# wheretrue/exon

Measured on AMD Instinct MI355X. Metric: Mrows/sec filter+agg on 1B-row synthetic VCF; achieved HBM GB/s vs peak, higher is better.
Workload: dtype f64

## Files before the change

exon_amd/csrc/kernels.h:

```cpp
#pragma once
#include <hip/hip_runtime.h>
#include <stdint.h>

namespace exon {

struct Workspace {
  unsigned long long* partials = nullptr;
  size_t partial_capacity = 0;
  int* status = nullptr;
  uint2* tail_rec_a = nullptr;
  uint2* tail_rec_b = nullptr;
  size_t tail_capacity = 0;
  unsigned* tail_u32 = nullptr;
};

struct LaunchCfg {
  int compute_units = 256;
  int blocks_per_cu = 8;
  bool overwrite = false;
  bool x_is_int = false;
  bool y_is_int = false;
};

size_t k2_partial_words(const LaunchCfg&);
// ... 14 lines not shown
                                int64_t region_start, int64_t region_end, int64_t* d_count, bool strict = false);

hipError_t launch_flag_mapq_group_count(hipStream_t s, const LaunchCfg& cfg, const Workspace& ws, const int32_t* flag,
                                        const uint8_t* flag_valid, const uint8_t* mapq, const uint8_t* mapq_valid,
                                        const int32_t* ref_id, const uint8_t* ref_valid, int64_t n, int32_t flag_mask,
                                        int32_t flag_value, int32_t mapq_min, int32_t n_refs, int64_t* d_counts);

hipError_t launch_cmp_avg_by_group(hipStream_t s, const LaunchCfg& cfg, const Workspace& ws, const float* x,
                                   const uint8_t* x_valid, const float* y, const uint8_t* y_valid, const int32_t* gid,
                                   int64_t n, double thr, int cmp_op, int n_groups, int64_t* d_counts, double* d_sums);

hipError_t launch_cmp_minmax_by_group(hipStream_t s, const LaunchCfg& cfg, const Workspace& ws, const float* x,
                                      const uint8_t* x_valid, const float* y, const uint8_t* y_valid, const int32_t* gid,
                                      int64_t n, double thr, int cmp_op, int n_groups, int64_t* d_state);

hipError_t launch_qual_pos_hist(hipStream_t s, const LaunchCfg& cfg, const Workspace& ws, const int32_t* offsets,
                                const uint8_t* bytes, int64_t n_reads, int lmax, int64_t* d_hist);
hipError_t launch_qual_pos_hist_views(hipStream_t s, const LaunchCfg& cfg, const Workspace& ws, const int32_t* starts,
                                      const int32_t* ends, const uint8_t* bytes, int64_t n_reads, int lmax,
                                      int64_t* d_hist);

constexpr int K5_MAX_CHUNKS = 64;
struct K5Chunks {
  const int32_t* off[K5_MAX_CHUNKS];
  const int32_t* ends[K5_MAX_CHUNKS];
  const uint8_t* bytes[K5_MAX_CHUNKS];
  int64_t n[K5_MAX_CHUNKS];
  int count;
};
hipError_t launch_qual_pos_hist_chunks(hipStream_t s, const LaunchCfg& cfg, const Workspace& ws, const K5Chunks& ch, int lmax,
                                       int64_t* d_hist);

constexpr int K9_LEN_LDS = 8192;
constexpr int64_t read_stats_words(int lmax) { return 4 + ((int64_t)lmax + 1) + 102 + 257; }
hipError_t launch_read_stats_hist(hipStream_t s, const LaunchCfg& cfg, const Workspace& ws, const uint8_t* sbytes, const int32_t* ss,
                                  const int32_t* se, const uint8_t* qbytes, const int32_t* qs, const int32_t* qe, int64_t n_reads, int lmax,
                                  int64_t* d_state);

hipError_t launch_region_mask(hipStream_t s, bool range_form, const int32_t* id_col, const uint8_t* id_valid, const int64_t* start,
                              const int64_t* end, const uint8_t* pos_valid, const uint8_t* in_valid, int64_t n, int32_t id,
                              int64_t a, int64_t b, uint8_t* out_valid, unsigned long long* n_pass);

hipError_t launch_value_mask(hipStream_t s, const void* x, const uint8_t* x_valid, bool x_is_int, double literal, int cmp_op, const uint8_t* region_mask,
                             const uint8_t* in_valid, int64_t n, uint8_t* out_valid, unsigned long long* n_pass);

hipError_t launch_flag_mapq_mask(hipStream_t s, const int32_t* flag, const uint8_t* mapq, const uint8_t* mapq_valid, int32_t flag_mask, int32_t flag_value,
                                 int32_t mapq_min, const uint8_t* region_mask, const uint8_t* in_valid, int64_t n, uint8_t* out_valid, unsigned long long* n_pass);

hipError_t launch_fold_states(hipStream_t s, const void* gathered, int world, int64_t n_i64, int64_t n_f64, void* out, int64_t n_max = 0);

hipError_t launch_permute_add_state(hipStream_t s, const void* src, void* dst, const int32_t* map, int n_map, int G, int planes_i64,
                                    int tail_i64, int planes_f64, int planes_max);

hipError_t launch_read_probe(hipStream_t s, const LaunchCfg& cfg, const void* const* buffers, int n_buffers, int64_t bytes_each,
                             unsigned* sink);

hipError_t launch_gen_c2(hipStream_t s, uint64_t seed, int64_t n_total, int64_t lo, int64_t hi, int32_t* chrom,
                         int64_t* pos);
hipError_t launch_gen_c3(hipStream_t s, uint64_t seed, int64_t lo, int64_t hi, int32_t* flag, uint8_t* mapq,
                         uint8_t* mapq_valid, int32_t* ref_id, uint8_t* ref_valid);
hipError_t launch_gen_c4(hipStream_t s, uint64_t seed, int64_t lo, int64_t hi, float* af, uint8_t* af_valid,
                         float* qual, uint8_t* qual_valid, int32_t* filter_id);
hipError_t launch_gen_c6(hipStream_t s, uint64_t seed, int64_t lo, int64_t hi, int32_t* ref_id, uint8_t* ref_valid,
                         int64_t* start, int64_t* end, uint8_t* pos_valid);
hipError_t launch_gen_c5(hipStream_t s, uint64_t seed, int64_t lo, int64_t hi, int32_t read_len, int32_t* offsets,
                         uint8_t* bytes);

}
```

exon_amd/csrc/kernels.hip:

```cpp
#include "kernels.h"
#include "host/cmp_key.h"

#include <algorithm>
#include <cstdlib>
#include <cstring>
#include <mutex>
#include <type_traits>

namespace exon {

struct ShapeBig {
  static constexpr int THREADS = 1024, J = 4;
};
struct ShapeSmall {
  static constexpr int THREADS = 256, J = 2;
};
struct ShapeBigJ2 {
  static constexpr int THREADS = 1024, J = 2;
};
template <typename S>
struct ShapeOf {
  static constexpr int WAVES = S::THREADS / 64;
  static constexpr int WAVE_TILE = 256 * S::J;
  static constexpr int TILE = WAVES * WAVE_TILE;
// ... 209 lines not shown
    for (int r = 0; r < world; ++r) t = max(t, gathered[(size_t)r * V + v]);
    out[v] = t;
  } else if (v < n_i64) {
    unsigned long long t = 0;
    for (int r = 0; r < world; ++r) t += gathered[(size_t)r * V + v];
    out[v] = t;
  } else {
    double t = 0.0;
    for (int r = 0; r < world; ++r) t += __longlong_as_double((long long)gathered[(size_t)r * V + v]);
    out[v] = (unsigned long long)__double_as_longlong(t);
  }
}

hipError_t launch_fold_states(hipStream_t s, const void* gathered, int world, int64_t n_i64, int64_t n_f64, void* out, int64_t n_max) {
  const int64_t V = n_i64 + n_f64;
  if (V <= 0 || world < 1 || n_max < 0 || n_max > n_i64) return hipErrorInvalidValue;
  hipLaunchKernelGGL(fold_states, dim3((unsigned)((V + 255) / 256)), dim3(256), 0, s,
                     static_cast<const unsigned long long*>(gathered), world, (int)V, (int)n_i64, (int)n_max,
                     static_cast<unsigned long long*>(out));
  return hipGetLastError();
}

__global__ __launch_bounds__(256) void permute_add_state(const unsigned long long* __restrict__ src, unsigned long long* __restrict__ dst,
                                                         const int32_t* __restrict__ map, int n_map, int G, int planes_i64, int tail_i64,
                                                         int planes_f64, int planes_max) {
  const int g = blockIdx.x * 256 + threadIdx.x;
  if (g < tail_i64) {
    const size_t w = (size_t)planes_i64 * G + g;
    if (src[w]) atomicAdd(&dst[w], src[w]);
  }
  if (g >= n_map || g >= G) return;
  const int t = map[g];
  if (t < 0 || t >= G) return;
  for (int p = 0; p < planes_i64; ++p) {
    const unsigned long long v = src[(size_t)p * G + g];
    if (!v) continue;
    if (p >= planes_i64 - planes_max) atomicMax(&dst[(size_t)p * G + t], v);
    else atomicAdd(&dst[(size_t)p * G + t], v);
  }
  const size_t fbase = (size_t)planes_i64 * G + tail_i64;
  for (int p = 0; p < planes_f64; ++p) {
    const double v = __longlong_as_double((long long)src[fbase + (size_t)p * G + g]);
    if (v != 0.0) atomicAdd(reinterpret_cast<double*>(dst) + fbase + (size_t)p * G + t, v);
  }
}

hipError_t launch_permute_add_state(hipStream_t s, const void* src, void* dst, const int32_t* map, int n_map, int G, int planes_i64,
                                    int tail_i64, int planes_f64, int planes_max) {
  if (G < 0 || n_map < 0 || planes_i64 < 0 || planes_f64 < 0 || tail_i64 < 0 || planes_max < 0 || planes_max > planes_i64) return hipErrorInvalidValue;
  const int threads = std::max(std::min(n_map, G), tail_i64);
  if (threads == 0) return hipSuccess;
  hipLaunchKernelGGL(permute_add_state, dim3((unsigned)((threads + 255) / 256)), dim3(256), 0, s, static_cast<const unsigned long long*>(src),
                     static_cast<unsigned long long*>(dst), map, n_map, G, planes_i64, tail_i64, planes_f64, planes_max);
  return hipGetLastError();
}

template <typename F>
static int resident_blocks(F f, int threads, size_t lds) {
  int nb = 0;
  if (hipOccupancyMaxActiveBlocksPerMultiprocessor(&nb, f, threads, lds) != hipSuccess || nb < 1) nb = 1;
  return nb;
}

static bool use_big_shape(const LaunchCfg& cfg, int64_t n) {
  const int64_t cus = std::max(cfg.compute_units, 1);
  return n / ShapeOf<ShapeBigJ2>::TILE >= cus;
}

template <typename S>
static int grid_for(const LaunchCfg& cfg, int64_t n, int resident) {
  const int64_t tiles = (n + ShapeOf<S>::TILE - 1) / ShapeOf<S>::TILE;
  const int per_cu = S::THREADS >= 1024 ? 1 : std::min(cfg.blocks_per_cu, resident);
  int64_t g = (int64_t)cfg.compute_units * per_cu;
  if (g > tiles) g = tiles;
  if (g < 1) g = 1;
  return (int)g;
}
static int max_grid(const LaunchCfg& cfg) { return cfg.compute_units * std::max(cfg.blocks_per_cu, 1); }

template <int NB>
__global__ __launch_bounds__(ShapeBig::THREADS) void k_read_probe(const uint4* __restrict__ b0, const uint4* __restrict__ b1,
                                                                  const uint4* __restrict__ b2, const uint4* __restrict__ b3,
                                                                  int64_t nvec, unsigned* __restrict__ sink) {
  using S = ShapeBig;
  constexpr int J = S::J, WAVES = ShapeOf<S>::WAVES, WT = 64 * J, TILE = WAVES * WT;
  const int lane = threadIdx.x & 63, wave = threadIdx.x >> 6;
  const uint4* const bufs[4] = {b0, b1, b2, b3};
  uint4 acc = uint4{0, 0, 0, 0};
  const int64_t ntiles = nvec / TILE;
  for (int64_t tile = blockIdx.x; tile < ntiles; tile += gridDim.x) {
    const int64_t wbase = tile * TILE + (int64_t)wave * WT;
    uint4 v[NB][J];
#pragma unroll
    for (int j = 0; j < J; ++j)
#pragma unroll
      for (int b = 0; b < NB; ++b) v[b][j] = ld16<uint4>(bufs[b] + wbase + j * 64 + lane);
#pragma unroll
    for (int j = 0; j < J; ++j)
#pragma unroll
      for (int b = 0; b < NB; ++b) {
        acc.x += v[b][j].x;
        acc.y += v[b][j].y;
        acc.z += v[b][j].z;
        acc.w += v[b][j].w;
      }
  }
// ... 2548 lines not shown
```

exon_amd/csrc/stream.cpp:

```cpp
#include <hip/hip_runtime.h>

#include <dlfcn.h>
#include <time.h>

#include <algorithm>
#include <atomic>
#include <condition_variable>
#include <cstdio>
#include <cstdlib>
#include <chrono>
#include <cstring>
#include <deque>
#include <memory>
#include <mutex>
#include <new>
#include <functional>
#include <string>
#include <thread>
#include <unordered_map>
#include <vector>

#include "host/arrow_build.h"
#include "host/bitmap.h"
#include "host/raw_batch.h"
#include "internal.h"

namespace {

struct ColSpec {
  int elem = 4;
  bool utf8 = false;
};

struct ColStage {
  uint8_t* h_values = nullptr;
  uint8_t* h_valid = nullptr;
  int32_t* h_offsets = nullptr;
  uint8_t* d_values = nullptr;
  uint8_t* d_valid = nullptr;
  int32_t* d_offsets = nullptr;
  bool any_null_bitmap = false;
  int64_t bytes = 0;
};

struct CopySpan {
  uint8_t* dst;
  const uint8_t* src;
  size_t n;
};
struct HeldBatch {
  struct ArrowArray array;
  const struct ArrowArray* ch[4];
  int64_t off[4];
  int64_t rows, row0;
};
struct Slot {
  std::vector<ColStage> cols;
  int64_t rows = 0;
  hipEvent_t done = nullptr;
  bool in_flight = false;
  std::vector<HeldBatch> held;
  size_t submitted = 0;
  int64_t unsubmitted_bytes = 0;
  std::vector<std::unique_ptr<std::vector<CopySpan>>> span_runs;
  std::atomic<size_t> pending{0};
};

}

struct exon_hip_plan {
  exon_hip_ctx* ctx;
  exon_hip_plan_desc d;
  int64_t n_i64, n_f64;
  int64_t n_max = 0;
  int n_cols;
  ColSpec cols[4];
};

struct exon_hip_stream {
  exon_hip_plan* plan;
  exon_hip_ctx* ctx;
  hipStream_t stream = nullptr;
  uint8_t* d_state = nullptr;
  Slot slots[2];
  int cur = 0;
  int64_t cap_rows = 0, cap_bytes = 0;
  bool closed = false;
  int64_t rows_pushed = 0;
  double t_copy = 0, t_wait = 0, t_enqueue = 0;
  bool overwrite_next = false;
  int x_type = -1, y_type = -1;
  std::function<int32_t()> null_group;
  uint8_t* d_gather = nullptr;
  size_t gather_bytes = 0;
  std::vector<std::string> keys;
  int keys_state = 0;
  uint8_t* d_rekey_state = nullptr;
  int32_t* d_map = nullptr;
  size_t map_cap = 0;
  uint8_t* saved_state = nullptr;
  bool saved_overwrite = false;
  std::string region_contig;
  bool has_region_contig = false;
  int32_t region_id_override = INT32_MIN;
};
enum { KEYS_NONE = 0, KEYS_LOCAL = 1, KEYS_AGREED = 2 };
constexpr size_t COLL_SCRATCH = 8192;
constexpr int64_t HOLD_MAX_ROWS = 1 << 17;

static bool key_layout(const exon_hip_plan* p, int* G, int* planes_i, int* tail, int* planes_f, int* planes_max) {
  *planes_max = 0;
  switch (p->d.kind) {
    case EXON_HIP_PLAN_FLAG_MAPQ_GROUP_COUNT:
      *G = p->d.n_groups, *planes_i = 1, *tail = 1, *planes_f = 0;
      return true;
    case EXON_HIP_PLAN_CMP_AVG_BY_GROUP:
      *G = p->d.n_groups, *planes_i = 2, *tail = 0, *planes_f = 1;
      return true;
    case EXON_HIP_PLAN_CMP_MINMAX_BY_GROUP:
      *G = p->d.n_groups, *planes_i = 4, *tail = 0, *planes_f = 0, *planes_max = 2;
      return true;
  }
  return false;
}

namespace {
class CopyPool {
 public:
  static CopyPool& get() {
    static CopyPool p;
    return p;
  }
  typedef CopySpan Span;
  void submit(const Span* v, size_t count, std::atomic<size_t>* left) {
    if (threads_.empty()) {
      for (size_t i = 0; i < count; ++i) memcpy(v[i].dst, v[i].src, v[i].n);
      return;
    }
    {
      std::lock_guard<std::mutex> g(mu_);
      size_t i = 0;
      while (i < count) {
        size_t j = i, bytes = 0;
        while (j < count && bytes < (1u << 20)) bytes += v[j++].n;
        left->fetch_add(1, std::memory_order_relaxed);
        jobs_.push_back(Job{nullptr, reinterpret_cast<const uint8_t*>(v + i), j - i, left});
        i = j;
      }
    }
    cv_.notify_all();
  }
  void help_until(std::atomic<size_t>* left) {
    while (left->load(std::memory_order_acquire) != 0) {
      Job j;
      bool have = false;
      {
        std::lock_guard<std::mutex> g(mu_);
        if (!jobs_.empty()) {
          j = jobs_.front();
          jobs_.pop_front();
          have = true;
        }
      }
      if (have) do_job(j);
      else std::this_thread::yield();
    }
  }
  void copy(void* dst, const void* src, size_t n) {
    constexpr size_t PIECE = 1u << 20;
    if (threads_.empty() || n < 4 * PIECE) {
      memcpy(dst, src, n);
      return;
    }
    std::atomic<size_t> left{0};
    size_t pieces = 0;
    {
      std::lock_guard<std::mutex> g(mu_);
      for (size_t o = 0; o < n; o += PIECE) {
        jobs_.push_back(Job{static_cast<uint8_t*>(dst) + o, static_cast<const uint8_t*>(src) + o, std::min(PIECE, n - o), &left});
        ++pieces;
      }
      left.store(pieces, std::memory_order_relaxed);
    }
    cv_.notify_all();
    for (;;) {
      Job j;
      {
        std::lock_guard<std::mutex> g(mu_);
        if (jobs_.empty()) break;
        j = jobs_.front();
        jobs_.pop_front();
      }
      do_job(j);
    }
    while (left.load(std::memory_order_acquire) != 0) std::this_thread::yield();
  }

 private:
  struct Job {
    uint8_t* dst;
    const uint8_t* src;
    size_t n;
    std::atomic<size_t>* left;
  };
  static void do_job(const Job& j) {
    if (j.dst) {
      memcpy(j.dst, j.src, j.n);
    } else {
      const Span* v = reinterpret_cast<const Span*>(j.src);
      for (size_t i = 0; i < j.n; ++i) memcpy(v[i].dst, v[i].src, v[i].n);
    }
    j.left->fetch_sub(1, std::memory_order_acq_rel);
  }
  CopyPool() {
    int t = 8;
    if (const char* v = getenv("EXON_HIP_STAGE_THREADS")) t = atoi(v);
    const int hc = (int)std::thread::hardware_concurrency();
    if (hc > 0) t = std::min(t, std::max(1, hc / 2));
    int dev = 0;
    const void* cpus = hipGetDevice(&dev) == hipSuccess ? exon_hip_gpu_local_cpus(dev) : nullptr;
    for (int i = 1; i < t; ++i)
      threads_.emplace_back([this, cpus] {
        exon_hip_run_on(cpus);
        run();
      });
  }
  ~CopyPool() {
    {
      std::lock_guard<std::mutex> g(mu_);
      stop_ = true;
    }
    cv_.notify_all();
    for (auto& th : threads_) th.join();
  }
  void run() {
    for (;;) {
      Job j;
      {
        std::unique_lock<std::mutex> lk(mu_);
        cv_.wait(lk, [this] { return stop_ || !jobs_.empty(); });
        if (stop_) return;
        j = jobs_.front();
        jobs_.pop_front();
      }
      do_job(j);
    }
  }
  std::mutex mu_;
  std::condition_variable cv_;
  std::deque<Job> jobs_;
  std::vector<std::thread> threads_;
  bool stop_ = false;
};
}

using exon::append_bits;

static double now_s() {
  struct timespec ts;
  clock_gettime(CLOCK_MONOTONIC, &ts);
  return (double)ts.tv_sec + 1e-9 * (double)ts.tv_nsec;
}

static void free_slot(Slot& s) {
  CopyPool::get().help_until(&s.pending);
  for (auto& h : s.held)
    if (h.array.release) h.array.release(&h.array);
  s.held.clear();
  s.span_runs.clear();
  s.submitted = 0;
  s.unsubmitted_bytes = 0;
  for (auto& c : s.cols) {
    if (c.h_values) hipHostFree(c.h_values);
    if (c.h_valid) hipHostFree(c.h_valid);
    if (c.h_offsets) hipHostFree(c.h_offsets);
    if (c.d_values) hipFree(c.d_values);
    if (c.d_valid) hipFree(c.d_valid);
    if (c.d_offsets) hipFree(c.d_offsets);
  }
  s.cols.clear();
  if (s.done) hipEventDestroy(s.done);
  s.done = nullptr;
}

static int alloc_slot(exon_hip_stream* st, Slot& s) {
  exon_hip_plan* p = st->plan;
  s.cols.assign((size_t)p->n_cols, ColStage());
  for (int c = 0; c < p->n_cols; ++c) {
    ColStage& cs = s.cols[(size_t)c];
    const size_t vbytes = p->cols[c].utf8 ? (size_t)st->cap_bytes : (size_t)st->cap_rows * (size_t)p->cols[c].elem;
    const size_t bbytes = (size_t)(st->cap_rows + 7) / 8 + 64;
    if (hipHostMalloc((void**)&cs.h_values, vbytes + 64) != hipSuccess) return EXON_HIP_ENOMEM;
    if (hipMalloc((void**)&cs.d_values, vbytes + 64) != hipSuccess) return EXON_HIP_ENOMEM;
    if (hipHostMalloc((void**)&cs.h_valid, bbytes) != hipSuccess) return EXON_HIP_ENOMEM;
    if (hipMalloc((void**)&cs.d_valid, bbytes) != hipSuccess) return EXON_HIP_ENOMEM;
    memset(cs.h_valid, 0, bbytes);
    if (p->cols[c].utf8) {
      const size_t ob = ((size_t)st->cap_rows + 1) * 4;
      if (hipHostMalloc((void**)&cs.h_offsets, ob) != hipSuccess) return EXON_HIP_ENOMEM;
      if (hipMalloc((void**)&cs.d_offsets, ob) != hipSuccess) return EXON_HIP_ENOMEM;
      cs.h_offsets[0] = 0;
    }
  }
  if (!s.done && hipEventCreateWithFlags(&s.done, hipEventDisableTiming) != hipSuccess) return EXON_HIP_EDEVICE;
  s.rows = 0;
  s.in_flight = false;
  return EXON_HIP_OK;
}

static int run_plan(const exon_hip_plan* p, void* stream, const exon_hip_column* cols, int64_t n, int flags, void* d_state, int x_type = -1,
                    int y_type = -1, int32_t region_id = INT32_MIN) {
  exon_hip_plan_desc d = p->d;
  if (region_id != INT32_MIN) d.region_chrom_id = region_id;
  if (x_type < 0) x_type = d.x_type;
  if (y_type < 0) y_type = d.y_type;
  if (x_type == EXON_HIP_X_INT32) flags |= EXON_LAUNCH_X_INT32;
  if (y_type == EXON_HIP_X_INT32) flags |= EXON_LAUNCH_Y_INT32;
  exon_hip_ctx* ctx = p->ctx;
  int64_t* counts = reinterpret_cast<int64_t*>(d_state);
  double* sums = reinterpret_cast<double*>(static_cast<uint8_t*>(d_state) + p->n_i64 * 8);
  switch (d.kind) {
    case EXON_HIP_PLAN_REGION_COUNT:
      return exon_op_region_count(ctx, stream, &cols[0], &cols[1], n, d.region_chrom_id, d.region_start, d.region_end, counts,
                                  flags);
    case EXON_HIP_PLAN_FLAG_MAPQ_GROUP_COUNT:
      return exon_op_flag_mapq_group_count(ctx, stream, &cols[0], &cols[1], &cols[2], n, d.flag_mask, d.flag_value, d.mapq_min,
                                           d.n_groups, counts, flags);
    case EXON_HIP_PLAN_CMP_AVG_BY_GROUP:
      return exon_op_cmp_avg_by_group(ctx, stream, &cols[0], &cols[1], &cols[2], n, d.threshold, d.cmp_op, d.n_groups, counts,
                                      sums, flags);
    case EXON_HIP_PLAN_CMP_MINMAX_BY_GROUP:
      return exon_op_cmp_minmax_by_group(ctx, stream, &cols[0], &cols[1], &cols[2], n, d.threshold, d.cmp_op, d.n_groups, counts,
                                         flags);
    case EXON_HIP_PLAN_QUAL_POS_HIST:
      return exon_op_qual_pos_hist(ctx, stream, &cols[0], n, d.lmax, counts, flags);
    case EXON_HIP_PLAN_READ_STATS_HIST:
      return exon_op_read_stats_hist(ctx, stream, &cols[0], &cols[1], n, d.lmax, counts, flags);
    case EXON_HIP_PLAN_OVERLAP_COUNT:
    case EXON_HIP_PLAN_WITHIN_COUNT:
      return exon_op_overlap_count(ctx, stream, &cols[0], &cols[1], &cols[2], n, d.region_chrom_id, d.region_start,
                                   d.region_end, counts, flags, d.kind == EXON_HIP_PLAN_WITHIN_COUNT);
  }
  return fail(ctx, EXON_HIP_EINVAL, "unknown plan kind %d", d.kind);
}
static int launch_plan(exon_hip_stream* st, const exon_hip_column* cols, int64_t n) {
  const int flags = st->overwrite_next ? EXON_HIP_LAUNCH_OVERWRITE : EXON_HIP_LAUNCH_ACCUMULATE;
  int rc = run_plan(st->plan, st->stream, cols, n, flags, st->d_state, st->x_type, st->y_type, st->region_id_override);
  if (!rc) st->overwrite_next = false;
  return rc;
}
static int settle_reset(exon_hip_stream* st) {
  if (!st->overwrite_next) return EXON_HIP_OK;
  HIP_TRY(st->ctx, hipMemsetAsync(st->d_state, 0, (size_t)(st->plan->n_i64 + st->plan->n_f64) * 8, st->stream));
  st->overwrite_next = false;
  return EXON_HIP_OK;
}

static void release_held(Slot& s) {
  CopyPool::get().help_until(&s.pending);
  for (auto& h : s.held)
    if (h.array.release) h.array.release(&h.array);
  s.held.clear();
  s.span_runs.clear();
  s.submitted = 0;
  s.unsubmitted_bytes = 0;
}
static void submit_held(exon_hip_stream* st, Slot& s) {
  if (s.submitted == s.held.size()) return;
  exon_hip_plan* p = st->plan;
  auto run = std::make_unique<std::vector<CopySpan>>();
  run->reserve((s.held.size() - s.submitted) * (size_t)p->n_cols);
  for (size_t k = s.submitted; k < s.held.size(); ++k) {
    const HeldBatch& h = s.held[k];
    for (int c = 0; c < p->n_cols; ++c) {
      ColStage& cs = s.cols[(size_t)c];
      const int e = p->cols[c].elem;
      run->push_back(CopySpan{cs.h_values + (size_t)h.row0 * e, (const uint8_t*)h.ch[c]->buffers[1] + (size_t)h.off[c] * e, (size_t)h.rows * e});
      const uint8_t* valid = (const uint8_t*)h.ch[c]->buffers[0];
      if (valid && h.ch[c]->null_count != 0) {
        if (!cs.any_null_bitmap) {
          append_bits(cs.h_valid, 0, nullptr, 0, h.row0);
          cs.any_null_bitmap = true;
        }
        append_bits(cs.h_valid, h.row0, valid, h.off[c], h.rows);
      } else if (cs.any_null_bitmap) {
        append_bits(cs.h_valid, h.row0, nullptr, 0, h.rows);
      }
    }
  }
  CopyPool::get().submit(run->data(), run->size(), &s.pending);
  s.span_runs.push_back(std::move(run));
  s.submitted = s.held.size();
  s.unsubmitted_bytes = 0;
}
static void materialise_held(exon_hip_stream* st, Slot& s) {
  if (s.held.empty()) return;
  const double t_c0 = now_s();
  submit_held(st, s);
  release_held(s);
  st->t_copy += now_s() - t_c0;
}

static int flush_slot(exon_hip_stream* st) {
  Slot& s = st->slots[st->cur];
  if (s.rows == 0) return EXON_HIP_OK;
  materialise_held(st, s);
  exon_hip_plan* p = st->plan;
  const double t_f0 = now_s();
  exon_hip_column cols[4];
  for (int c = 0; c < p->n_cols; ++c) {
    ColStage& cs = s.cols[(size_t)c];
    const size_t vbytes = p->cols[c].utf8 ? (size_t)cs.bytes : (size_t)s.rows * (size_t)p->cols[c].elem;
    bool null_key_rewritten = false;
    if (cs.any_null_bitmap && c == 2 && (p->d.kind == EXON_HIP_PLAN_CMP_AVG_BY_GROUP || p->d.kind == EXON_HIP_PLAN_CMP_MINMAX_BY_GROUP) && st->null_group) {
      const int32_t id = st->null_group();
      if (id < 0) return fail(st->ctx, EXON_HIP_ESTATE, "the scan has no dictionary for its nullable group key");
      int32_t* ids = reinterpret_cast<int32_t*>(cs.h_values);
      for (int64_t i = 0; i < s.rows; ++i)
        if (!((cs.h_valid[i >> 3] >> (i & 7)) & 1)) ids[i] = id;
      null_key_rewritten = true;
    }
    if (vbytes) HIP_TRY(st->ctx, hipMemcpyAsync(cs.d_values, cs.h_values, vbytes, hipMemcpyHostToDevice, st->stream));
    cols[c].values = cs.d_values;
    cols[c].validity = nullptr;
    cols[c].offsets = nullptr;
    cols[c].length = s.rows;
    if (cs.any_null_bitmap && !null_key_rewritten) {
      HIP_TRY(st->ctx, hipMemcpyAsync(cs.d_valid, cs.h_valid, (size_t)(s.rows + 7) / 8, hipMemcpyHostToDevice, st->stream));
      cols[c].validity = cs.d_valid;
    }
    if (p->cols[c].utf8) {
      HIP_TRY(st->ctx, hipMemcpyAsync(cs.d_offsets, cs.h_offsets, ((size_t)s.rows + 1) * 4, hipMemcpyHostToDevice, st->stream));
      cols[c].offsets = cs.d_offsets;
    }
  }
  int rc = launch_plan(st, cols, s.rows);
  if (rc) return rc;
  HIP_TRY(st->ctx, hipEventRecord(s.done, st->stream));
  s.in_flight = true;
  const double t_f1 = now_s();
  st->t_enqueue += t_f1 - t_f0;
  st->cur ^= 1;
  Slot& n = st->slots[st->cur];
  if (n.in_flight) {
    HIP_TRY(st->ctx, hipEventSynchronize(n.done));
    n.in_flight = false;
  }
  st->t_wait += now_s() - t_f1;
  n.rows = 0;
  for (auto& cs : n.cols) {
    cs.bytes = 0;
    if (cs.any_null_bitmap) memset(cs.h_valid, 0, (size_t)(st->cap_rows + 7) / 8 + 64);
    cs.any_null_bitmap = false;
    if (cs.h_offsets) cs.h_offsets[0] = 0;
  }
  return EXON_HIP_OK;
}

static int ensure_capacity(exon_hip_stream* st, int64_t rows, int64_t bytes) {
  if (st->cap_rows >= rows && st->cap_bytes >= bytes && !st->slots[0].cols.empty()) return EXON_HIP_OK;
  int rc = flush_slot(st);
  if (rc) return rc;
  HIP_TRY(st->ctx, hipStreamSynchronize(st->stream));
  for (auto& s : st->slots) free_slot(s);
  int64_t def_rows = 4 << 20, def_bytes = 256ll << 20;
  if (const char* v = getenv("EXON_HIP_COALESCE_ROWS")) {
    long long x = atoll(v);
    if (x >= 1) def_rows = x;
  }
  st->cap_rows = std::max(st->cap_rows, std::max(rows, def_rows));
  st->cap_bytes = std::max(st->cap_bytes, std::max(bytes, def_bytes));
  for (auto& s : st->slots)
    if ((rc = alloc_slot(st, s))) return fail(st->ctx, rc, "staging allocation failed (%lld rows)", (long long)st->cap_rows);
  st->cur = 0;
  return EXON_HIP_OK;
}

extern "C" {

int exon_hip_plan_create(exon_hip_ctx* ctx, const exon_hip_plan_desc* desc, exon_hip_plan** out) {
  if (!ctx || !desc || !out) return fail(ctx, EXON_HIP_EINVAL, "exon_hip_plan_create: NULL argument");
  *out = nullptr;
  exon_hip_plan* p = new (std::nothrow) exon_hip_plan();
  if (!p) return fail(ctx, EXON_HIP_ENOMEM, "out of host memory");
  p->ctx = ctx;
  p->d = *desc;
  p->n_i64 = p->n_f64 = 0;
  switch (desc->kind) {
// ... 35 lines not shown
    case EXON_HIP_PLAN_CMP_MINMAX_BY_GROUP:
      p->n_cols = 3;
      p->cols[0].elem = p->cols[1].elem = p->cols[2].elem = 4;
      if (desc->n_groups < 1 || desc->n_groups > EXON_HIP_MAX_GROUPS) {
        delete p;
        return fail(ctx, EXON_HIP_EUNSUPPORTED, "n_groups %d outside [1, %d]", desc->n_groups, EXON_HIP_MAX_GROUPS);
      }
      if (desc->cmp_op < EXON_HIP_GT || desc->cmp_op > EXON_HIP_NE) {
        delete p;
        return fail(ctx, EXON_HIP_EINVAL, "bad cmp_op %d", desc->cmp_op);
      }
      p->n_i64 = 4 * desc->n_groups;
      p->n_max = 2 * desc->n_groups;
      break;
    case EXON_HIP_PLAN_OVERLAP_COUNT:
      p->n_cols = 3;
      p->cols[0].elem = 4;
      p->cols[1].elem = p->cols[2].elem = 8;
      p->n_i64 = 1;
      if (desc->region_start < 1 || desc->region_end < desc->region_start) {
        delete p;
        return fail(ctx, EXON_HIP_EINVAL, "region interval must satisfy 1 <= start <= end");
      }
      break;
    case EXON_HIP_PLAN_WITHIN_COUNT:
      p->n_cols = 3;
      p->cols[0].elem = 4;
      p->cols[1].elem = p->cols[2].elem = 8;
      p->n_i64 = 1;
      break;
    case EXON_HIP_PLAN_QUAL_POS_HIST:
      p->n_cols = 1;
      p->cols[0].elem = 1;
      p->cols[0].utf8 = true;
      if (desc->lmax < 1 || desc->lmax > 65536) {
        delete p;
        return fail(ctx, EXON_HIP_EINVAL, "lmax %d out of range", desc->lmax);
      }
      p->n_i64 = (int64_t)desc->lmax * 256;
      break;
    case EXON_HIP_PLAN_READ_STATS_HIST:
      p->n_cols = 2;
      p->cols[0].elem = p->cols[1].elem = 1;
      p->cols[0].utf8 = p->cols[1].utf8 = true;
      if (desc->lmax < 1 || desc->lmax > 65536) {
        delete p;
        return fail(ctx, EXON_HIP_EINVAL, "lmax %d out of range", desc->lmax);
      }
      p->n_i64 = 4 + ((int64_t)desc->lmax + 1) + 102 + 257;
      break;
    default:
      delete p;
      return fail(ctx, EXON_HIP_EINVAL, "unknown plan kind %d", desc->kind);
  }
  for (int c = 0; c < p->n_cols; ++c)
    if (desc->columns[c] < 0) {
      delete p;
      return fail(ctx, EXON_HIP_EINVAL, "negative column index");
    }
  *out = p;
  return EXON_HIP_OK;
}

int exon_hip_plan_destroy(exon_hip_plan* plan) {
  delete plan;
  return EXON_HIP_OK;
}

int exon_hip_plan_state_size(const exon_hip_plan* plan, int64_t* n_i64, int64_t* n_f64) {
  if (!plan || !n_i64 || !n_f64) return fail(nullptr, EXON_HIP_EINVAL, "exon_hip_plan_state_size: NULL argument");
  *n_i64 = plan->n_i64;
  *n_f64 = plan->n_f64;
  return EXON_HIP_OK;
}

int exon_hip_stream_open(exon_hip_plan* plan, int32_t partition, exon_hip_stream** out) {
  (void)partition;
  if (!plan || !out) return fail(plan ? plan->ctx : nullptr, EXON_HIP_EINVAL, "exon_hip_stream_open: NULL argument");
  *out = nullptr;
  exon_hip_ctx* ctx = plan->ctx;
  exon_hip_stream* st = new (std::nothrow) exon_hip_stream();
  if (!st) return fail(ctx, EXON_HIP_ENOMEM, "out of host memory");
  st->plan = plan;
  st->ctx = ctx;
  hipSetDevice(ctx->device);
  hipError_t e;
  const size_t sbytes = (size_t)(plan->n_i64 + plan->n_f64) * 8;
  int prio_least = 0, prio_greatest = 0;
  const char* pv = getenv("EXON_HIP_STREAM_PRIORITY");
  const bool use_prio = !(pv && pv[0] == '0') && hipDeviceGetStreamPriorityRange(&prio_least, &prio_greatest) == hipSuccess && prio_least != prio_greatest;
  if ((e = use_prio ? hipStreamCreateWithPriority(&st->stream, hipStreamNonBlocking, prio_greatest)
                    : hipStreamCreateWithFlags(&st->stream, hipStreamNonBlocking)) != hipSuccess ||
      (e = hipMalloc((void**)&st->d_state, ((sbytes + 63) & ~(size_t)63) + COLL_SCRATCH)) != hipSuccess ||
      (e = hipMemsetAsync(st->d_state, 0, sbytes, st->stream)) != hipSuccess) {
    if (st->stream) hipStreamDestroy(st->stream);
    if (st->d_state) hipFree(st->d_state);
    delete st;
    return fail(ctx, EXON_HIP_EDEVICE, "stream open: %s", hipGetErrorString(e));
  }
  *out = st;
  return EXON_HIP_OK;
}

static int column_child(exon_hip_stream* st, const struct ArrowArray* batch, int c, const struct ArrowArray** child,
                        int64_t* eff_off) {
  const int idx = st->plan->d.columns[c];
// ... 12 lines not shown
  *child = ch;
  return EXON_HIP_OK;
}

int exon_hip_stream_push(exon_hip_stream* st, struct ArrowArray* batch) {
  if (!st || !batch) return fail(st ? st->ctx : nullptr, EXON_HIP_EINVAL, "exon_hip_stream_push: NULL argument");
  if (!batch->release) return fail(st->ctx, EXON_HIP_EINVAL, "batch already released");
  if (st->closed) {
    batch->release(batch);
    return fail(st->ctx, EXON_HIP_ESTATE, "push after finish/close");
  }
  exon_hip_plan* p = st->plan;
  const int64_t rows = batch->length;
  int rc = EXON_HIP_OK;
  const struct ArrowArray* ch[4];
  int64_t off[4];
  int64_t need_bytes = 0, col_bytes[4] = {0, 0, 0, 0};
  for (int c = 0; c < p->n_cols && !rc; ++c) {
    rc = column_child(st, batch, c, &ch[c], &off[c]);
    if (!rc && p->cols[c].utf8 && rows > 0) {
      const int32_t* o = (const int32_t*)ch[c]->buffers[1];
      col_bytes[c] = (int64_t)o[off[c] + rows] - o[off[c]];
      need_bytes = std::max<int64_t>(need_bytes, col_bytes[c]);
    }
  }
  if (!rc && rows > 0) {
    rc = ensure_capacity(st, rows, need_bytes);
    if (!rc) {
      const Slot& cur = st->slots[st->cur];
      bool full = cur.rows + rows > st->cap_rows;
      for (int c = 0; c < p->n_cols; ++c) full = full || cur.cols[(size_t)c].bytes + col_bytes[c] > st->cap_bytes;
      if (full) rc = flush_slot(st);
    }
    bool fixed = true;
    for (int c = 0; c < p->n_cols; ++c) fixed = fixed && !p->cols[c].utf8;
    static const bool hold_on = [] {
      const char* v = getenv("EXON_HIP_HOLD_SMALL_BATCHES");
      return !(v && v[0] == '0');
    }();
    if (!rc && fixed && hold_on && rows <= HOLD_MAX_ROWS) {
      Slot& s = st->slots[st->cur];
      HeldBatch h;
      h.array = *batch;
      batch->release = nullptr;
      for (int c = 0; c < p->n_cols; ++c) {
        h.ch[c] = ch[c];
        h.off[c] = off[c];
      }
      h.rows = rows;
      h.row0 = s.rows;
      s.held.push_back(h);
      s.rows += rows;
      st->rows_pushed += rows;
      for (int c = 0; c < p->n_cols; ++c) s.unsubmitted_bytes += rows * p->cols[c].elem;
      if (s.unsubmitted_bytes >= (4 << 20)) submit_held(st, s);
      return EXON_HIP_OK;
    }
    if (!rc) {
      Slot& s = st->slots[st->cur];
      materialise_held(st, s);
      const double t_c0 = now_s();
      for (int c = 0; c < p->n_cols; ++c) {
        ColStage& cs = s.cols[(size_t)c];
        const uint8_t* valid = (const uint8_t*)ch[c]->buffers[0];
        if (valid && ch[c]->null_count != 0) {
          if (!cs.any_null_bitmap) {
            append_bits(cs.h_valid, 0, nullptr, 0, s.rows);
            cs.any_null_bitmap = true;
          }
          append_bits(cs.h_valid, s.rows, valid, off[c], rows);
        } else if (cs.any_null_bitmap) {
          append_bits(cs.h_valid, s.rows, nullptr, 0, rows);
        }
        if (p->cols[c].utf8) {
          const int32_t* o = (const int32_t*)ch[c]->buffers[1] + off[c];
          const uint8_t* data = (const uint8_t*)ch[c]->buffers[2];
          const int32_t base = o[0], len = o[rows] - base;
          if (len) CopyPool::get().copy(cs.h_values + cs.bytes, data + base, (size_t)len);
          const int32_t shift = (int32_t)cs.bytes - base;
          for (int64_t i = 1; i <= rows; ++i) cs.h_offsets[s.rows + i] = o[i] + shift;
          cs.bytes += len;
        } else {
          const int e = p->cols[c].elem;
          CopyPool::get().copy(cs.h_values + (size_t)s.rows * e, (const uint8_t*)ch[c]->buffers[1] + (size_t)off[c] * e, (size_t)rows * e);
        }
      }
      s.rows += rows;
      st->rows_pushed += rows;
      st->t_copy += now_s() - t_c0;
    }
  }
  batch->release(batch);
  return rc;
}

}

int exon_hip_stream_launch_scan_columns(exon_hip_stream* st, const exon_hip_column* scan_cols, int n_scan_cols, int64_t n,
                                        const uint8_t* row_mask) {
  exon_hip_plan* p = st->plan;
  if (st->closed) return fail(st->ctx, EXON_HIP_ESTATE, "push after finish/close");
  int rc = flush_slot(st);
  if (rc) return rc;
  exon_hip_column cols[4];
  for (int c = 0; c < p->n_cols; ++c) {
    const int idx = p->d.columns[c];
    if (idx >= n_scan_cols || !scan_cols[idx].values) return fail(st->ctx, EXON_HIP_EINVAL, "plan needs scan column %d which this scan does not produce", idx);
    cols[c] = scan_cols[idx];
  }
  if (row_mask) cols[0].validity = row_mask;
  rc = launch_plan(st, cols, n);
  if (!rc) st->rows_pushed += n;
  return rc;
}
int exon_hip_stream_plan_first_column(exon_hip_stream* st) { return st->plan->d.columns[0]; }
int exon_hip_stream_plan_kind(exon_hip_stream* st) { return st->plan->d.kind; }
int exon_hip_stream_plan_column(exon_hip_stream* st, int arg) { return arg >= 0 && arg < st->plan->n_cols ? st->plan->d.columns[arg] : -1; }
int exon_hip_stream_set_value_types(exon_hip_stream* st, int x_type, int y_type) {
  if (st->plan->d.kind == EXON_HIP_PLAN_CMP_MINMAX_BY_GROUP && st->rows_pushed > 0) {
    const int held = st->y_type >= 0 ? st->y_type : st->plan->d.y_type;
    if (held != y_type)
      return fail(st->ctx, EXON_HIP_ESTATE,
                  "the stream's MIN / MAX state holds %s values and this file's header types the argument %s: one stream takes one type "
                  "(finish it and open another for this file)", held == EXON_HIP_X_INT32 ? "Int32" : "Float32", y_type == EXON_HIP_X_INT32 ? "Int32" : "Float32");
  }
  st->x_type = x_type;
  st->y_type = y_type;
  return EXON_HIP_OK;
}
int exon_hip_stream_set_null_group(exon_hip_stream* st, std::function<int32_t()> id_of_null) {
  int rc = EXON_HIP_OK;
  if (!id_of_null && st->null_group && !st->closed) rc = flush_slot(st);
  st->null_group = std::move(id_of_null);
  return rc;
}
int exon_hip_stream_launch_views(exon_hip_stream* st, const uint8_t* d_text, const exon_hip_fastq_views& v) {
  exon_hip_plan* p = st->plan;
// ... 10 lines not shown
  if (rc) return rc;
  (void)d_text;
  if (k9) {
    rc = exon_hip_read_stats_hist_views(st->ctx, st->stream, v.text_base, v.seq_start, v.seq_end, v.qual_start, v.qual_end, v.n_reads, p->d.lmax,
                                        reinterpret_cast<int64_t*>(st->d_state));
    if (!rc) st->rows_pushed += v.n_reads;
    return rc;
  }
  rc = exon_hip_qual_pos_hist_views(st->ctx, st->stream, v.text_base, idx == 2 ? v.seq_start : v.qual_start,
                                    idx == 2 ? v.seq_end : v.qual_end, v.n_reads, p->d.lmax,
                                    reinterpret_cast<int64_t*>(st->d_state));
  if (!rc) st->rows_pushed += v.n_reads;
  return rc;
}
void* exon_hip_stream_hip_stream(exon_hip_stream* st) { return (void*)st->stream; }
exon_hip_ctx* exon_hip_stream_ctx(exon_hip_stream* st) { return st->ctx; }
int exon_hip_stream_state_copy(exon_hip_stream* st, void* d_snapshot, bool restore, int64_t* rows_pushed) {
  if (!restore) {
    int rc = flush_slot(st);
    if (!rc) rc = settle_reset(st);
    if (rc) return rc;
    if (rows_pushed) *rows_pushed = st->rows_pushed;
  } else {
    st->overwrite_next = false;
    if (rows_pushed) st->rows_pushed = *rows_pushed;
  }
  const size_t bytes = (size_t)(st->plan->n_i64 + st->plan->n_f64) * 8;
  HIP_TRY(st->ctx, hipMemcpyAsync(restore ? (void*)st->d_state : d_snapshot, restore ? d_snapshot : (void*)st->d_state, bytes,
                                  hipMemcpyDeviceToDevice, st->stream));
  return EXON_HIP_OK;
}
size_t exon_hip_stream_state_bytes(exon_hip_stream* st) { return (size_t)(st->plan->n_i64 + st->plan->n_f64) * 8; }

int exon_hip_stream_push_raw(exon_hip_stream* st, const exon::RawBatch& rb) {
  exon_hip_plan* p = st->plan;
  if (st->closed) return fail(st->ctx, EXON_HIP_ESTATE, "push after finish/close");
  for (int c = 0; c < p->n_cols; ++c) {
    if (p->cols[c].utf8) return fail(st->ctx, EXON_HIP_EUNSUPPORTED, "raw push of a Utf8 column");
    const int idx = p->d.columns[c];
    if (idx >= (int)rb.cols.size()) return fail(st->ctx, EXON_HIP_EINVAL, "scan has %zu columns, plan needs index %d", rb.cols.size(), idx);
    if (rb.cols[(size_t)idx].elem != p->cols[c].elem) return fail(st->ctx, EXON_HIP_EINVAL, "column %d: element size %d, plan expects %d", idx, rb.cols[(size_t)idx].elem, p->cols[c].elem);
  }
  int64_t done = 0;
  while (done < rb.rows) {
    int rc = ensure_capacity(st, 1, 0);
    if (rc) return rc;
    if (st->slots[st->cur].rows >= st->cap_rows && (rc = flush_slot(st))) return rc;
    Slot& s = st->slots[st->cur];
    materialise_held(st, s);
    const int64_t n = std::min<int64_t>(rb.rows - done, st->cap_rows - s.rows);
    for (int c = 0; c < p->n_cols; ++c) {
      const exon::RawColumn& rc2 = rb.cols[(size_t)p->d.columns[c]];
      ColStage& cs = s.cols[(size_t)c];
      const int e = p->cols[c].elem;
      CopyPool::get().copy(cs.h_values + (size_t)s.rows * e, static_cast<const uint8_t*>(rc2.values) + (size_t)done * e, (size_t)n * e);
      if (rc2.valid_bytes) {
        if (!cs.any_null_bitmap) {
          append_bits(cs.h_valid, 0, nullptr, 0, s.rows);
          cs.any_null_bitmap = true;
        }
        const uint8_t* v = rc2.valid_bytes + done;
        for (int64_t i = 0; i < n; ++i)
          if (v[i]) cs.h_valid[(s.rows + i) >> 3] |= (uint8_t)(1u << ((s.rows + i) & 7));
      } else if (cs.any_null_bitmap) {
        append_bits(cs.h_valid, s.rows, nullptr, 0, n);
      }
    }
    s.rows += n;
    st->rows_pushed += n;
    done += n;
  }
  return EXON_HIP_OK;
}

extern "C" {

int exon_hip_stream_push_device(exon_hip_stream* st, const struct ArrowDeviceArray* dbatch) {
  if (!st || !dbatch) return fail(st ? st->ctx : nullptr, EXON_HIP_EINVAL, "exon_hip_stream_push_device: NULL argument");
  if (st->closed) return fail(st->ctx, EXON_HIP_ESTATE, "push after finish/close");
  if (dbatch->device_type != ARROW_DEVICE_ROCM)
    return fail(st->ctx, EXON_HIP_EINVAL, "device_type %d is not ARROW_DEVICE_ROCM", (int)dbatch->device_type);
  if (dbatch->device_id != st->ctx->device)
    return fail(st->ctx, EXON_HIP_EINVAL, "batch lives on device %lld, stream on %d", (long long)dbatch->device_id, st->ctx->device);
  exon_hip_plan* p = st->plan;
  const struct ArrowArray* batch = &dbatch->array;
  const int64_t rows = batch->length;
  exon_hip_column cols[4];
  for (int c = 0; c < p->n_cols; ++c) {
    const struct ArrowArray* ch;
    int64_t off;
    int rc = column_child(st, batch, c, &ch, &off);
    if (rc) return rc;
    cols[c].length = rows;
    cols[c].validity = nullptr;
    cols[c].offsets = nullptr;
    if (ch->buffers[0] && ch->null_count != 0) {
      if (off & 7) return fail(st->ctx, EXON_HIP_EINVAL, "device batch: validity bit offset must be a multiple of 8");
      cols[c].validity = (const uint8_t*)ch->buffers[0] + (off >> 3);
    }
    if (p->cols[c].utf8) {
      cols[c].offsets = (const int32_t*)ch->buffers[1] + off;
      cols[c].values = ch->buffers[2];
    } else {
      cols[c].values = (const uint8_t*)ch->buffers[1] + (size_t)off * p->cols[c].elem;
    }
  }
  if (dbatch->sync_event) HIP_TRY(st->ctx, hipStreamWaitEvent(st->stream, *(hipEvent_t*)dbatch->sync_event, 0));
  int rc = launch_plan(st, cols, rows);
// ... 915 lines not shown
```

Baseline: 554,400.

## Stage group-id column as u8/u16 on host and widen on device

For the group-by plans, the int32 group-key column is now narrowed to 1 or 2 bytes while it is copied into pinned host staging, transferred over the bus in that narrow form, and widened back to int32 by a new GPU kernel before the plan runs. Out-of-range ids map to a sentinel. The aim is to cut host-to-device transfer bytes and staging memcpy volume for that column, which matters when the stream is transfer-bound. In exchange it adds a per-element narrowing loop on the host copy threads, an extra device kernel and buffer, and id remapping for the sentinel and null cases. It can be disabled with an environment variable.

```diff
diff --git a/exon_amd/csrc/host/narrow_ids.h b/exon_amd/csrc/host/narrow_ids.h
--- /dev/null
+++ b/exon_amd/csrc/host/narrow_ids.h
@@ -0,0 +1,27 @@
+#pragma once
+#include <stddef.h>
+#include <stdint.h>
+
+namespace exon {
+
+inline int narrow_id_bytes(int64_t n_groups) { return n_groups <= 255 ? 1 : n_groups <= 65535 ? 2 : 4; }
+
+typedef int32_t __attribute__((aligned(1), may_alias)) narrow_src_i32;
+
+template <typename T>
+inline void narrow_ids(T* __restrict__ dst, const void* __restrict__ src_, size_t rows, uint32_t n_groups) {
+  static_assert(sizeof(T) == 1 || sizeof(T) == 2, "u8 or u16");
+  const narrow_src_i32* __restrict__ src = static_cast<const narrow_src_i32*>(src_);
+  constexpr uint32_t SENTINEL = sizeof(T) == 1 ? 0xFFu : 0xFFFFu;
+  for (size_t i = 0; i < rows; ++i) {
+    const uint32_t v = (uint32_t)src[i];
+    dst[i] = (T)(v < n_groups ? v : SENTINEL);
+  }
+}
+
+inline void narrow_ids_to(int staged_bytes, void* dst, const void* src, size_t rows, uint32_t n_groups) {
+  if (staged_bytes == 1) narrow_ids(static_cast<uint8_t*>(dst), src, rows, n_groups);
+  else narrow_ids(static_cast<uint16_t*>(dst), src, rows, n_groups);
+}
+
+}
diff --git a/exon_amd/csrc/kernels.h b/exon_amd/csrc/kernels.h
--- a/exon_amd/csrc/kernels.h
+++ b/exon_amd/csrc/kernels.h
@@ -90,6 +90,8 @@
 hipError_t launch_permute_add_state(hipStream_t s, const void* src, void* dst, const int32_t* map, int n_map, int G, int planes_i64,
                                     int tail_i64, int planes_f64, int planes_max);
 
+hipError_t launch_widen_ids(hipStream_t s, const void* narrow, int id_bytes, int32_t* ids, int64_t rows);
+
 hipError_t launch_read_probe(hipStream_t s, const LaunchCfg& cfg, const void* const* buffers, int n_buffers, int64_t bytes_each,
                              unsigned* sink);
 
diff --git a/exon_amd/csrc/kernels.hip b/exon_amd/csrc/kernels.hip
--- a/exon_amd/csrc/kernels.hip
+++ b/exon_amd/csrc/kernels.hip
@@ -285,6 +285,36 @@
   if (threads == 0) return hipSuccess;
   hipLaunchKernelGGL(permute_add_state, dim3((unsigned)((threads + 255) / 256)), dim3(256), 0, s, static_cast<const unsigned long long*>(src),
                      static_cast<unsigned long long*>(dst), map, n_map, G, planes_i64, tail_i64, planes_f64, planes_max);
+  return hipGetLastError();
+}
+
+template <typename T>
+__global__ __launch_bounds__(256) void k_widen_ids(const T* __restrict__ src, int32_t* __restrict__ dst, int64_t rows) {
+  const int64_t quads = rows >> 2;
+  const int64_t stride = (int64_t)gridDim.x * 256;
+  for (int64_t q = (int64_t)blockIdx.x * 256 + threadIdx.x; q < quads; q += stride) {
+    int4 o;
+    if constexpr (sizeof(T) == 1) {
+      const uint32_t w = reinterpret_cast<const uint32_t*>(src)[q];
+      o = make_int4((int)(w & 0xFFu), (int)((w >> 8) & 0xFFu), (int)((w >> 16) & 0xFFu), (int)(w >> 24));
+    } else {
+      const uint2 w = reinterpret_cast<const uint2*>(src)[q];
+      o = make_int4((int)(w.x & 0xFFFFu), (int)(w.x >> 16), (int)(w.y & 0xFFFFu), (int)(w.y >> 16));
+    }
+    reinterpret_cast<int4*>(dst)[q] = o;
+  }
+  if (blockIdx.x == 0 && (int64_t)threadIdx.x < (rows & 3)) {
+    const int64_t i = (quads << 2) + threadIdx.x;
+    dst[i] = (int32_t)src[i];
+  }
+}
+
+hipError_t launch_widen_ids(hipStream_t s, const void* narrow, int id_bytes, int32_t* ids, int64_t rows) {
+  if (rows < 0 || (id_bytes != 1 && id_bytes != 2)) return hipErrorInvalidValue;
+  if (rows == 0) return hipSuccess;
+  const int64_t blocks = std::min<int64_t>(std::max<int64_t>(((rows >> 2) + 255) / 256, 1), 16384);
+  if (id_bytes == 1) hipLaunchKernelGGL(k_widen_ids<uint8_t>, dim3((unsigned)blocks), dim3(256), 0, s, static_cast<const uint8_t*>(narrow), ids, rows);
+  else hipLaunchKernelGGL(k_widen_ids<uint16_t>, dim3((unsigned)blocks), dim3(256), 0, s, static_cast<const uint16_t*>(narrow), ids, rows);
   return hipGetLastError();
 }
 
diff --git a/exon_amd/csrc/stream.cpp b/exon_amd/csrc/stream.cpp
--- a/exon_amd/csrc/stream.cpp
+++ b/exon_amd/csrc/stream.cpp
@@ -22,6 +22,7 @@
 
 #include "host/arrow_build.h"
 #include "host/bitmap.h"
+#include "host/narrow_ids.h"
 #include "host/raw_batch.h"
 #include "internal.h"
 
@@ -29,7 +30,9 @@
 
 struct ColSpec {
   int elem = 4;
+  int stage = 4;
   bool utf8 = false;
+  uint32_t n_groups = 0;
 };
 
 struct ColStage {
@@ -37,6 +40,7 @@
   uint8_t* h_valid = nullptr;
   int32_t* h_offsets = nullptr;
   uint8_t* d_values = nullptr;
+  uint8_t* d_narrow = nullptr;
   uint8_t* d_valid = nullptr;
   int32_t* d_offsets = nullptr;
   bool any_null_bitmap = false;
@@ -47,7 +51,19 @@
   uint8_t* dst;
   const uint8_t* src;
   size_t n;
+  int narrow;
+  uint32_t n_groups;
 };
+inline void stage_span(const CopySpan& s) {
+  if (s.narrow) exon::narrow_ids_to(s.narrow, s.dst, s.src, s.n, s.n_groups);
+  else memcpy(s.dst, s.src, s.n);
+}
+inline CopySpan stage_span_of(const ColSpec& c, uint8_t* h_values, int64_t row0, const void* src, int64_t src_row0, int64_t rows) {
+  const uint8_t* from = static_cast<const uint8_t*>(src) + (size_t)src_row0 * c.elem;
+  uint8_t* to = h_values + (size_t)row0 * c.stage;
+  if (c.stage != c.elem) return CopySpan{to, from, (size_t)rows, c.stage, c.n_groups};
+  return CopySpan{to, from, (size_t)rows * c.elem, 0, 0};
+}
 struct HeldBatch {
   struct ArrowArray array;
   const struct ArrowArray* ch[4];
@@ -134,7 +150,7 @@
   typedef CopySpan Span;
   void submit(const Span* v, size_t count, std::atomic<size_t>* left) {
     if (threads_.empty()) {
-      for (size_t i = 0; i < count; ++i) memcpy(v[i].dst, v[i].src, v[i].n);
+      for (size_t i = 0; i < count; ++i) stage_span(v[i]);
       return;
     }
     {
@@ -142,9 +158,9 @@
       size_t i = 0;
       while (i < count) {
         size_t j = i, bytes = 0;
-        while (j < count && bytes < (1u << 20)) bytes += v[j++].n;
+        while (j < count && bytes < (1u << 20)) bytes += src_bytes(v[j++]);
         left->fetch_add(1, std::memory_order_relaxed);
-        jobs_.push_back(Job{nullptr, reinterpret_cast<const uint8_t*>(v + i), j - i, left});
+        jobs_.push_back(Job{Span{}, v + i, j - i, left});
         i = j;
       }
     }
@@ -166,18 +182,21 @@
       else std::this_thread::yield();
     }
   }
-  void copy(void* dst, const void* src, size_t n) {
+  void copy(void* dst, const void* src, size_t n) { stage(Span{static_cast<uint8_t*>(dst), static_cast<const uint8_t*>(src), n, 0, 0}); }
+  void stage(const Span& sp) {
     constexpr size_t PIECE = 1u << 20;
-    if (threads_.empty() || n < 4 * PIECE) {
-      memcpy(dst, src, n);
+    if (threads_.empty() || src_bytes(sp) < 4 * PIECE) {
+      stage_span(sp);
       return;
     }
+    const size_t unit = sp.narrow ? PIECE / 4 : PIECE;
+    const size_t dst_unit = sp.narrow ? (size_t)sp.narrow : 1, src_unit = sp.narrow ? 4 : 1;
     std::atomic<size_t> left{0};
     size_t pieces = 0;
     {
       std::lock_guard<std::mutex> g(mu_);
-      for (size_t o = 0; o < n; o += PIECE) {
-        jobs_.push_back(Job{static_cast<uint8_t*>(dst) + o, static_cast<const uint8_t*>(src) + o, std::min(PIECE, n - o), &left});
+      for (size_t o = 0; o < sp.n; o += unit) {
+        jobs_.push_back(Job{Span{sp.dst + o * dst_unit, sp.src + o * src_unit, std::min(unit, sp.n - o), sp.narrow, sp.n_groups}, nullptr, 0, &left});
         ++pieces;
       }
       left.store(pieces, std::memory_order_relaxed);
@@ -198,18 +217,16 @@
 
  private:
   struct Job {
-    uint8_t* dst;
-    const uint8_t* src;
-    size_t n;
+    Span one;
+    const Span* run;
+    size_t count;
     std::atomic<size_t>* left;
   };
+  static size_t src_bytes(const Span& s) { return s.narrow ? s.n * 4 : s.n; }
   static void do_job(const Job& j) {
-    if (j.dst) {
-      memcpy(j.dst, j.src, j.n);
-    } else {
-      const Span* v = reinterpret_cast<const Span*>(j.src);
-      for (size_t i = 0; i < j.n; ++i) memcpy(v[i].dst, v[i].src, v[i].n);
-    }
+    if (!j.run) stage_span(j.one);
+    else
+      for (size_t i = 0; i < j.count; ++i) stage_span(j.run[i]);
     j.left->fetch_sub(1, std::memory_order_acq_rel);
   }
   CopyPool() {
@@ -275,6 +292,7 @@
     if (c.h_valid) hipHostFree(c.h_valid);
     if (c.h_offsets) hipHostFree(c.h_offsets);
     if (c.d_values) hipFree(c.d_values);
+    if (c.d_narrow) hipFree(c.d_narrow);
     if (c.d_valid) hipFree(c.d_valid);
     if (c.d_offsets) hipFree(c.d_offsets);
   }
@@ -289,9 +307,11 @@
   for (int c = 0; c < p->n_cols; ++c) {
     ColStage& cs = s.cols[(size_t)c];
     const size_t vbytes = p->cols[c].utf8 ? (size_t)st->cap_bytes : (size_t)st->cap_rows * (size_t)p->cols[c].elem;
+    const size_t sbytes = p->cols[c].utf8 ? (size_t)st->cap_bytes : (size_t)st->cap_rows * (size_t)p->cols[c].stage;
     const size_t bbytes = (size_t)(st->cap_rows + 7) / 8 + 64;
-    if (hipHostMalloc((void**)&cs.h_values, vbytes + 64) != hipSuccess) return EXON_HIP_ENOMEM;
+    if (hipHostMalloc((void**)&cs.h_values, sbytes + 64) != hipSuccess) return EXON_HIP_ENOMEM;
     if (hipMalloc((void**)&cs.d_values, vbytes + 64) != hipSuccess) return EXON_HIP_ENOMEM;
+    if (p->cols[c].stage != p->cols[c].elem && hipMalloc((void**)&cs.d_narrow, sbytes + 64) != hipSuccess) return EXON_HIP_ENOMEM;
     if (hipHostMalloc((void**)&cs.h_valid, bbytes) != hipSuccess) return EXON_HIP_ENOMEM;
     if (hipMalloc((void**)&cs.d_valid, bbytes) != hipSuccess) return EXON_HIP_ENOMEM;
     memset(cs.h_valid, 0, bbytes);
@@ -374,8 +394,7 @@
     const HeldBatch& h = s.held[k];
     for (int c = 0; c < p->n_cols; ++c) {
       ColStage& cs = s.cols[(size_t)c];
-      const int e = p->cols[c].elem;
-      run->push_back(CopySpan{cs.h_values + (size_t)h.row0 * e, (const uint8_t*)h.ch[c]->buffers[1] + (size_t)h.off[c] * e, (size_t)h.rows * e});
+      run->push_back(stage_span_of(p->cols[c], cs.h_values, h.row0, h.ch[c]->buffers[1], h.off[c], h.rows));
       const uint8_t* valid = (const uint8_t*)h.ch[c]->buffers[0];
       if (valid && h.ch[c]->null_count != 0) {
         if (!cs.any_null_bitmap) {
@@ -410,17 +429,24 @@
   exon_hip_column cols[4];
   for (int c = 0; c < p->n_cols; ++c) {
     ColStage& cs = s.cols[(size_t)c];
-    const size_t vbytes = p->cols[c].utf8 ? (size_t)cs.bytes : (size_t)s.rows * (size_t)p->cols[c].elem;
+    const size_t vbytes = p->cols[c].utf8 ? (size_t)cs.bytes : (size_t)s.rows * (size_t)p->cols[c].stage;
     bool null_key_rewritten = false;
     if (cs.any_null_bitmap && c == 2 && (p->d.kind == EXON_HIP_PLAN_CMP_AVG_BY_GROUP || p->d.kind == EXON_HIP_PLAN_CMP_MINMAX_BY_GROUP) && st->null_group) {
       const int32_t id = st->null_group();
       if (id < 0) return fail(st->ctx, EXON_HIP_ESTATE, "the scan has no dictionary for its nullable group key");
-      int32_t* ids = reinterpret_cast<int32_t*>(cs.h_values);
+      const int w = p->cols[c].stage;
+      const uint32_t idw = w == 4 || (uint32_t)id < p->cols[c].n_groups ? (uint32_t)id : 0xFFFFFFFFu;
       for (int64_t i = 0; i < s.rows; ++i)
-        if (!((cs.h_valid[i >> 3] >> (i & 7)) & 1)) ids[i] = id;
+        if (!((cs.h_valid[i >> 3] >> (i & 7)) & 1)) {
+          if (w == 4) reinterpret_cast<int32_t*>(cs.h_values)[i] = id;
+          else if (w == 2) reinterpret_cast<uint16_t*>(cs.h_values)[i] = (uint16_t)idw;
+          else cs.h_values[i] = (uint8_t)idw;
+        }
       null_key_rewritten = true;
     }
-    if (vbytes) HIP_TRY(st->ctx, hipMemcpyAsync(cs.d_values, cs.h_values, vbytes, hipMemcpyHostToDevice, st->stream));
+    if (vbytes) {
+      HIP_TRY(st->ctx, hipMemcpyAsync(cs.d_narrow ? cs.d_narrow : cs.d_values, cs.h_values, vbytes, hipMemcpyHostToDevice, st->stream));
+    }
     cols[c].values = cs.d_values;
     cols[c].validity = nullptr;
     cols[c].offsets = nullptr;
@@ -434,6 +460,9 @@
       cols[c].offsets = cs.d_offsets;
     }
   }
+  for (int c = 0; c < p->n_cols; ++c)
+    if (s.cols[(size_t)c].d_narrow)
+      HIP_TRY(st->ctx, exon::launch_widen_ids(st->stream, s.cols[(size_t)c].d_narrow, p->cols[c].stage, reinterpret_cast<int32_t*>(s.cols[(size_t)c].d_values), s.rows));
   int rc = launch_plan(st, cols, s.rows);
   if (rc) return rc;
   HIP_TRY(st->ctx, hipEventRecord(s.done, st->stream));
@@ -575,6 +604,15 @@
     default:
       delete p;
       return fail(ctx, EXON_HIP_EINVAL, "unknown plan kind %d", desc->kind);
+  }
+  for (int c = 0; c < p->n_cols; ++c) p->cols[c].stage = p->cols[c].elem;
+  if (desc->kind == EXON_HIP_PLAN_CMP_AVG_BY_GROUP || desc->kind == EXON_HIP_PLAN_CMP_MINMAX_BY_GROUP) {
+    static const bool narrow_on = [] {
+      const char* v = getenv("EXON_HIP_STAGE_NARROW_IDS");
+      return !(v && v[0] == '0');
+    }();
+    if (narrow_on) p->cols[2].stage = exon::narrow_id_bytes(desc->n_groups);
+    p->cols[2].n_groups = (uint32_t)desc->n_groups;
   }
   for (int c = 0; c < p->n_cols; ++c)
     if (desc->columns[c] < 0) {
@@ -693,7 +731,7 @@
       s.held.push_back(h);
       s.rows += rows;
       st->rows_pushed += rows;
-      for (int c = 0; c < p->n_cols; ++c) s.unsubmitted_bytes += rows * p->cols[c].elem;
+      for (int c = 0; c < p->n_cols; ++c) s.unsubmitted_bytes += rows * p->cols[c].stage;
       if (s.unsubmitted_bytes >= (4 << 20)) submit_held(st, s);
       return EXON_HIP_OK;
     }
@@ -722,8 +760,7 @@
           for (int64_t i = 1; i <= rows; ++i) cs.h_offsets[s.rows + i] = o[i] + shift;
           cs.bytes += len;
         } else {
-          const int e = p->cols[c].elem;
-          CopyPool::get().copy(cs.h_values + (size_t)s.rows * e, (const uint8_t*)ch[c]->buffers[1] + (size_t)off[c] * e, (size_t)rows * e);
+          CopyPool::get().stage(stage_span_of(p->cols[c], cs.h_values, s.rows, ch[c]->buffers[1], off[c], rows));
         }
       }
       s.rows += rows;
@@ -840,8 +877,7 @@
     for (int c = 0; c < p->n_cols; ++c) {
       const exon::RawColumn& rc2 = rb.cols[(size_t)p->d.columns[c]];
       ColStage& cs = s.cols[(size_t)c];
-      const int e = p->cols[c].elem;
-      CopyPool::get().copy(cs.h_values + (size_t)s.rows * e, static_cast<const uint8_t*>(rc2.values) + (size_t)done * e, (size_t)n * e);
+      CopyPool::get().stage(stage_span_of(p->cols[c], cs.h_values, s.rows, rc2.values, done, n));
       if (rc2.valid_bytes) {
         if (!cs.any_null_bitmap) {
           append_bits(cs.h_valid, 0, nullptr, 0, s.rows);
```

Result: no change. 556,800, median of 4 (+0.4%).
